# aquaskyline/SOAPdenovo-Trans

Hardware: AMD Instinct MI355X
Metric: pregraph k-mers hashed/sec (higher is better)
Workload: dtype u64

## Files before the change

soapdenovo-trans_amd/csrc/sdt_sk_scatter_seq.cuh:

```cuda
#pragma once
#include <hip/hip_runtime.h>
#include "sdt_kmer.cuh"
#include "sdt_table.cuh"
#include "sdt_superkmer.cuh"

using namespace sdt;

constexpr uint32_t SK_BLK = 128;
#ifndef SDT_SK_BLK2
#define SDT_SK_BLK2 1024
#endif
constexpr uint32_t SK_BLK2 = SDT_SK_BLK2;
constexpr uint32_t SK_DEAD = 0xFFFFFFFFu;

#ifdef SDT_SK_L2_LOG
extern __device__ unsigned long long *g_l2_log;
extern __device__ unsigned long long g_l2_log_cap;
__device__ inline void sk_log_alloc(uint32_t path, uint32_t end, uint32_t id)
{
	if (g_l2_log) {
		const unsigned long long at = atomicAdd(g_l2_log, 1ULL);
		if (at + 1 < g_l2_log_cap)
			g_l2_log[1 + at] = (1ULL << 63) | ((unsigned long long)path << 61) | ((unsigned long long)(threadIdx.x & 0x1FFF) << 48) |
			                   ((unsigned long long)(end & 0xFFFFFFu) << 24) | (unsigned long long)(id & 0xFFFFFFu);
	}
}
__device__ inline void sk_log_cursor(uint32_t kind, uint32_t lb, uint32_t chunk, uint32_t pos)
{
	if (g_l2_log) {
		const unsigned long long at = atomicAdd(g_l2_log, 1ULL);
		if (at + 1 < g_l2_log_cap)
			g_l2_log[1 + at] = (1ULL << 63) | (3ULL << 61) | ((unsigned long long)kind << 59) | ((unsigned long long)(blockIdx.x & 15u) << 55) |
			                   ((unsigned long long)(threadIdx.x & 1023u) << 45) | ((unsigned long long)(lb & 1023u) << 35) |
			                   ((unsigned long long)(pos > 31u ? 31u : pos) << 30) | (unsigned long long)(chunk & 0x3FFFFFFFu);
	}
}
#else
__device__ inline void sk_log_alloc(uint32_t, uint32_t, uint32_t) {}
__device__ inline void sk_log_cursor(uint32_t, uint32_t, uint32_t, uint32_t) {}
#endif

__device__ inline uint32_t sk_alloc_chunk(unsigned long long *s_blk, const SkPool &pool, uint32_t blk = SK_BLK)
{
	uint32_t got = 0;
	bool done = false;
	while (!done) {
		{
			const unsigned long long w = __hip_atomic_load(s_blk, __ATOMIC_RELAXED, __HIP_MEMORY_SCOPE_WORKGROUP);
			if ((uint32_t)w > (uint32_t)(w >> 32)) {
				__builtin_amdgcn_s_sleep(1);
				continue;
			}
		}
		const unsigned long long v = atomicAdd(s_blk, 1ULL);
		const uint32_t id = (uint32_t)v, end = (uint32_t)(v >> 32);
		if (id < end) {
			got = id;
			done = true;
			sk_log_alloc(0, end, id);
		} else if (id == end) {
			const uint32_t base = atomicAdd(pool.next, blk);
			atomicExch(s_blk, ((unsigned long long)(base + blk) << 32) | (unsigned long long)(base + 1u));
			got = base;
			done = true;
			sk_log_alloc(1, end, base);
		}
	}
	return got;
}

__device__ inline uint32_t sk_alloc_chunks(unsigned long long *s_blk, const SkPool &pool, uint32_t n, uint32_t blk)
{
	uint32_t got = SK_NOCHUNK;
	bool done = false;
	while (!done) {
		{
			const unsigned long long w = __hip_atomic_load(s_blk, __ATOMIC_RELAXED, __HIP_MEMORY_SCOPE_WORKGROUP);
			if ((uint32_t)w > (uint32_t)(w >> 32)) {
				__builtin_amdgcn_s_sleep(1);
				continue;
			}
		}
		const unsigned long long v = atomicAdd(s_blk, (unsigned long long)n);
		const uint32_t id = (uint32_t)v, end = (uint32_t)(v >> 32);
		if (id <= end && id + n <= end) {
			got = id;
			done = true;
		} else if (id <= end) {
			for (uint32_t x = id; x < end && x < pool.chunks; x++)
				pool.meta[x] = SK_DEAD;
			const uint32_t base = atomicAdd(pool.next, n + blk);
			atomicExch(s_blk, ((unsigned long long)(base + n + blk) << 32) | (unsigned long long)(base + n));
			got = base;
			done = true;
		}
	}
	return got;
}

__device__ inline void sk_retire_block(unsigned long long blk, const SkPool &pool)
{
	const uint32_t next = (uint32_t)blk, end = (uint32_t)(blk >> 32);
	for (uint32_t id = next; id < end && id < pool.chunks; id++)
		pool.meta[id] = SK_DEAD;
}

__device__ inline bool sk_reserve(unsigned long long *s_cur, unsigned long long *s_blk, uint32_t lb, uint32_t meta_bucket,
                                  uint32_t cap, const SkPool &pool, uint32_t *s_cnt, uint32_t &chunk, uint32_t &pos)
{
	bool done = false, ok = false;
	while (!done) {
		if ((uint32_t)__hip_atomic_load(&s_cur[lb], __ATOMIC_RELAXED, __HIP_MEMORY_SCOPE_WORKGROUP) > cap) {
			__builtin_amdgcn_s_sleep(1);
			continue;
		}
		const unsigned long long cur = atomicAdd(&s_cur[lb], 1ULL);
		pos = (uint32_t)cur;
		chunk = (uint32_t)(cur >> 32);
		if (pos < cap) {
			ok = chunk != SK_NOCHUNK;
			done = true;
			sk_log_cursor(0, lb, chunk, pos);
		} else if (pos == cap) {
			sk_log_cursor(1, lb, chunk, pos);
			uint32_t id = sk_alloc_chunk(s_blk, pool);
			if (id >= pool.chunks) {
				id = SK_NOCHUNK;
			} else {
				pool.meta[id] = meta_bucket | (cap << 24);
				atomicAdd(&s_cnt[lb], 1u);
			}
			atomicExch(&s_cur[lb], ((unsigned long long)id << 32) | 1ULL);
			chunk = id;
			pos = 0;
			ok = id != SK_NOCHUNK;
			done = true;
			sk_log_cursor(3, lb, id, 1);
		} else {
#if SDT_SK_L2_LOG >= 2
			sk_log_cursor(2, lb, chunk, pos);
#endif
		}
	}
	return ok;
}

template <int RW> __device__ inline void sk_store_record(uint64_t *dst, const uint64_t (&rec)[RW])
{
#pragma unroll
	for (int i = 0; i < RW; i++)
		dst[i] = rec[i];
}
template <int NW> __device__ inline void sk_store_record2(uint64_t *dst, const uint64_t (&rec)[SkFmt<NW>::REC_WORDS])
{
	if constexpr (SkFmt<NW>::REC2_STRIDE == 4 && SkFmt<NW>::REC_WORDS == 3) {
		ulonglong2 *d = reinterpret_cast<ulonglong2 *>(dst);
		d[0] = make_ulonglong2(rec[0], rec[1]);
		d[1] = make_ulonglong2(rec[2], 0ULL);
	} else {
		sk_store_record<SkFmt<NW>::REC_WORDS>(dst, rec);
	}
}
template <int RW> __device__ inline void sk_load_record(const uint64_t *src, uint64_t (&rec)[RW])
{
#pragma unroll
	for (int i = 0; i < RW; i++)
		rec[i] = src[i];
}


constexpr int SK_SEQ_TILE = 256;
constexpr int SK_SEQ_RUNCAP = 24;
constexpr int SK_SEQ_MAX_KMERS = 256;


template <int NW>
__device__ inline void sk_emit_run(const uint32_t *words, int rb_r, int len_r, int nk_r, int K, uint64_t read_ord, int j0, int n,
                                   uint32_t fb, unsigned long long *s_cur, unsigned long long *s_blk, const SkPool &pool,
                                   uint32_t *s_cnt, const Table<NW> &tbl, uint32_t &claimed, uint32_t &failed, uint32_t &done,
                                   uint32_t &emitted)
{
	constexpr int BW = SkFmt<NW>::BW, RW = SkFmt<NW>::REC_WORDS;
	const int hp = j0 > 0, hn = j0 + n < nk_r;
	const uint32_t l1 = fb >> SK_L2BITS, l2 = fb & (SK_NB2 - 1);
	uint32_t chunk, pos;
	if (sk_reserve(s_cur, s_blk, l1, l1, SK_CAP1, pool, s_cnt, chunk, pos)) {
		const int len = hp + n + K - 1 + hn, ps = rb_r + j0 - hp;
		uint64_t rec[RW];
		rec[0] = sk_header(read_ord, (uint32_t)j0, l2, n, hp, hn);
#pragma unroll
		for (int k = 0; k < BW; k++) {
			uint64_t wv = 0;
			if (32 * k < len) {
				wv = sk_stream_word(words, ps + 32 * k);
				const int keep = len - 32 * k;
				if (keep < 32)
					wv &= ~0ULL << (64 - 2 * keep);
			}
			rec[1 + k] = wv;
		}
		sk_store_record<RW>(pool.recs + ((size_t)chunk * SK_CAP1 + pos) * RW, rec);
		emitted += (uint32_t)n;
	} else if (!tbl.ent) {
		failed += (uint32_t)n;
	} else {
		for (int jj = j0; jj < j0 + n; jj++) {
			uint32_t prev, next;
			const Key<NW> key = chop_record<NW>(words, rb_r, len_r, jj, K, prev, next);
			const uint64_t ord = tbl.first ? (read_ord << 16) | (uint64_t)jj : ORD_NONE;
			if (!table_put<NW>(tbl, key, prev, next, claimed, ord))
				failed++;
			done++;
		}
	}
}

template <int NW, int W>
__global__ __launch_bounds__(SK_SEQ_TILE, NW == 1 ? 4 : 2) void k_sk_scatter_reads_seq(const uint32_t *__restrict__ packed, const uint64_t *__restrict__ offs,
                                                                      uint64_t nreads, int K, int m, int ncap, int max_tile_words, SkPool pool,
                                                                      unsigned long long *__restrict__ g_cursors, unsigned long long *__restrict__ g_blk,
                                                                      uint32_t *__restrict__ g_cnt, Table<NW> tbl, Stats *stats,
                                                                      uint64_t ord_base, uint64_t ord_stride)
{
	constexpr int TR = SK_SEQ_TILE;
	extern __shared__ uint32_t smem[];
	unsigned long long *s_cur = (unsigned long long *)smem;
	uint32_t *s_rb = (uint32_t *)(s_cur + SK_NB1);
	uint32_t *s_runs = s_rb + TR + 2;
	uint32_t *s_words = s_runs + TR * SK_SEQ_RUNCAP;
	__shared__ unsigned long long s_blk;
	__shared__ uint32_t s_cnt[SK_NB1];
	const int tid = threadIdx.x;
	for (int i = tid; i < SK_NB1; i += TR) {
		s_cur[i] = g_cursors[(size_t)blockIdx.x * SK_NB1 + i];
		s_cnt[i] = 0;
	}
	if (tid == 0)
		s_blk = g_blk[blockIdx.x];
	const uint64_t ntiles = (nreads + TR - 1) / TR;
	const uint32_t mmask = (1u << (2 * m)) - 1u;
	const int topsh = 2 * (m - 1);
	uint32_t claimed = 0, failed = 0, done = 0, emitted = 0;
#ifdef SDT_SK_TICKS
	unsigned long long cyc[4] = {0, 0, 0, 0}, t0 = wall_clock64(), t1;
#define SK_TICK(i) do { t1 = wall_clock64(); cyc[i] += t1 - t0; t0 = t1; } while (0)
#else
#define SK_TICK(i) do { } while (0)
#endif
	for (uint64_t tile = blockIdx.x; tile < ntiles; tile += gridDim.x) {
		const uint64_t r0 = tile * TR;
		const int nr = (int)((nreads - r0) < (uint64_t)TR ? (nreads - r0) : (uint64_t)TR);
		const uint64_t word0 = offs[r0] >> 4;
		int nwords = (int)(((offs[r0 + nr] + 15) >> 4) - word0) + TAIL_PAD;
		if (nwords > max_tile_words)
			nwords = max_tile_words;
		s_rb[tid] = (uint32_t)(offs[r0 + (tid < nr ? tid : nr)] - (word0 << 4));
		if (tid == 0)
			s_rb[TR] = (uint32_t)(offs[r0 + nr] - (word0 << 4));
		if (tid < LDS_LEAD)
			s_words[tid] = 0;
		for (int i = tid; i < nwords; i += TR)
			s_words[LDS_LEAD + i] = packed[word0 + i];
		__syncthreads();
		SK_TICK(0);
		const uint32_t *words = s_words + LDS_LEAD;
		const int rb_r = (int)s_rb[tid];
		const int len_r = tid < nr ? (int)s_rb[tid + 1] - rb_r : 0;
		const int nk_r = len_r >= K + 1 ? len_r - K + 1 : 0;
		const uint64_t read_ord = ord_base + (r0 + (uint64_t)tid) * ord_stride;
		uint32_t *runs = s_runs + tid * SK_SEQ_RUNCAP;
		int nrun = 0;
		if (nk_r > 0) {
			const int nhv = len_r - m + 1;
			uint32_t fw = sk_stream_mmer(words, rb_r, m) >> 2;
			uint32_t rc = (sk_rev2bit32(fw ^ 0xAAAAAAAAu) >> (32 - 2 * (m - 1))) << 2;
			int pb = rb_r + m - 1;
			auto next_hv = [&]() -> uint32_t {
				const uint32_t b = (words[pb >> 4] >> (30 - 2 * (pb & 15))) & 3u;
				pb++;
				fw = ((fw << 2) | b) & mmask;
				rc = (rc >> 2) | ((b ^ 2u) << topsh);
				return sk_mmer_hash(fw < rc ? fw : rc);
			};
			int j0 = 0;
			uint32_t fb0 = 0, pfb = 0;
			auto window = [&](int j, uint32_t mn) {
				const uint32_t fb = sk_final_bucket(sk_bucket_hash(mn));
				if (j == 0) {
					fb0 = fb;
				} else if (j - j0 >= ncap || fb != pfb) {
					if (nrun < SK_SEQ_RUNCAP)
						runs[nrun] = (fb0 << 6) | (uint32_t)(j - j0 - 1);
					else
						sk_emit_run<NW>(words, rb_r, len_r, nk_r, K, read_ord, j0, j - j0, fb0, s_cur, &s_blk, pool, s_cnt, tbl, claimed, failed, done, emitted);
					nrun++;
					j0 = j;
					fb0 = fb;
				}
				pfb = fb;
			};
			uint32_t h[W], nh[W];
#pragma clang loop unroll(full)
			for (int i = 0; i < W; i++)
				h[i] = next_hv();
#pragma clang loop unroll(full)
			for (int i = W - 2; i >= 0; i--)
				h[i] = h[i] < h[i + 1] ? h[i] : h[i + 1];
			int p = W;
			for (int jb = 0; jb < nk_r; jb += W) {
				window(jb, h[0]);
				uint32_t pre = 0xFFFFFFFFu;
#pragma clang loop unroll(full)
				for (int i = 1; i < W; i++) {
					const uint32_t x = p < nhv ? next_hv() : 0xFFFFFFFFu;
					p++;
					nh[i - 1] = x;
					pre = x < pre ? x : pre;
					if (jb + i < nk_r)
						window(jb + i, h[i] < pre ? h[i] : pre);
				}
				nh[W - 1] = p < nhv ? next_hv() : 0xFFFFFFFFu;
				p++;
				h[W - 1] = nh[W - 1];
#pragma clang loop unroll(full)
				for (int i = W - 2; i >= 0; i--)
					h[i] = nh[i] < h[i + 1] ? nh[i] : h[i + 1];
			}
			if (nrun < SK_SEQ_RUNCAP)
				runs[nrun] = (fb0 << 6) | (uint32_t)(nk_r - j0 - 1);
			else
				sk_emit_run<NW>(words, rb_r, len_r, nk_r, K, read_ord, j0, nk_r - j0, fb0, s_cur, &s_blk, pool, s_cnt, tbl, claimed, failed, done, emitted);
			nrun++;
		}
		SK_TICK(1);
		const int nlist = nrun < SK_SEQ_RUNCAP ? nrun : SK_SEQ_RUNCAP;
		for (int k = 0, jr = 0; k < nlist; k++) {
			const uint32_t e = runs[k];
			const int nr = (int)(e & 63u) + 1;
			sk_emit_run<NW>(words, rb_r, len_r, nk_r, K, read_ord, jr, nr, e >> 6, s_cur, &s_blk, pool, s_cnt, tbl, claimed, failed, done, emitted);
			jr += nr;
		}
		__syncthreads();
		SK_TICK(3);
	}
#undef SK_TICK
	for (int i = tid; i < SK_NB1; i += TR) {
		g_cursors[(size_t)blockIdx.x * SK_NB1 + i] = s_cur[i];
		if (s_cnt[i])
			atomicAdd(&g_cnt[i], s_cnt[i]);
	}
	if (tid == 0) {
		g_blk[blockIdx.x] = s_blk;
#ifdef SDT_SK_TICKS
		for (int i = 0; i < 4; i++)
			atomicAdd(&stats->sk_cyc1[i], cyc[i]);
#endif
	}
	if (done) {
		atomicAdd(&stats->kmers, (unsigned long long)done);
		atomicAdd(&stats->sk_direct, (unsigned long long)done);
	}
	if (claimed) atomicAdd(&stats->distinct, (unsigned long long)claimed);
	if (failed) atomicAdd(&stats->probe_fail, (unsigned long long)failed);
#pragma unroll
	for (int d = 32; d > 0; d >>= 1)
		emitted += __shfl_down(emitted, d);
	if ((tid & 63) == 0 && emitted)
		atomicAdd(&stats->sk_emitted, (unsigned long long)emitted);
}


struct SkSeqLaunch {
	const uint32_t *words;
	const uint64_t *offs;
	uint64_t nreads;
	int K, m, ncap, mtw;
	SkPool pool;
	unsigned long long *cursors, *blk;
	uint32_t *cnt;
	Stats *stats;
	uint64_t ord_base, ord_stride;
	unsigned max_wgs;
	int cu_count;
	hipStream_t stream;
};

template <int NW, int W> inline hipError_t sk_seq_launch_one(const SkSeqLaunch &a, const Table<NW> &tbl)
{
	const size_t smem = (size_t)SK_NB1 * 8 + (size_t)(SK_SEQ_TILE + 2) * 4 + (size_t)SK_SEQ_TILE * SK_SEQ_RUNCAP * 4 + (size_t)(LDS_LEAD + a.mtw) * 4;
	hipError_t e = hipFuncSetAttribute((const void *)k_sk_scatter_reads_seq<NW, W>, hipFuncAttributeMaxDynamicSharedMemorySize, (int)smem);
	if (e != hipSuccess) return e;
	int per_cu = 0;
	e = hipOccupancyMaxActiveBlocksPerMultiprocessor(&per_cu, k_sk_scatter_reads_seq<NW, W>, SK_SEQ_TILE, smem);
	if (e != hipSuccess) return e;
	uint64_t res = (uint64_t)(per_cu > 0 ? per_cu : 1) * (uint64_t)a.cu_count;
	if (res > a.max_wgs) res = a.max_wgs;
	const uint64_t nt = (a.nreads + SK_SEQ_TILE - 1) / SK_SEQ_TILE;
	const unsigned grid = (unsigned)(nt < res ? nt : res);
	hipLaunchKernelGGL((k_sk_scatter_reads_seq<NW, W>), dim3(grid), dim3(SK_SEQ_TILE), smem, a.stream, a.words, a.offs, a.nreads, a.K, a.m, a.ncap,
	                   a.mtw, a.pool, a.cursors, a.blk, a.cnt, tbl, a.stats, a.ord_base, a.ord_stride);
	return hipGetLastError();
}

hipError_t sk_seq_launch_nw1(int w, const SkSeqLaunch &a, const Table<1> &tbl);
hipError_t sk_seq_launch_nw2_lo(int w, const SkSeqLaunch &a, const Table<2> &tbl);
hipError_t sk_seq_launch_nw2_mid(int w, const SkSeqLaunch &a, const Table<2> &tbl);
hipError_t sk_seq_launch_nw2_hi(int w, const SkSeqLaunch &a, const Table<2> &tbl);
```

Measured before the change: 94.44 billion.

## Restructure super-k-mer walk with block base loads, 24-bit hash and warp-uniform windows

Reworks the per-read minimizer walk. Each block of W bases is now fetched with a few word loads and funnel shifts instead of one shared-memory load per base, and the m-mer hash is computed with 24-bit multiply-add instructions in inline assembly. The window loop uses a branch-free 'cut' scheme, with a full-block specialisation chosen when the whole warp agrees. Run-list overflow is handled by pausing the walk to flush the runs and then resuming, instead of emitting inline from inside the loop. The NW=2 launch bound is raised to 3 blocks per CU and the LDS tile is padded for over-reads, which may increase register pressure and changes the hash function's values.

```diff
diff --git a/soapdenovo-trans_amd/csrc/sdt_sk_scatter_seq.cuh b/soapdenovo-trans_amd/csrc/sdt_sk_scatter_seq.cuh
--- a/soapdenovo-trans_amd/csrc/sdt_sk_scatter_seq.cuh
+++ b/soapdenovo-trans_amd/csrc/sdt_sk_scatter_seq.cuh
@@ -1,5 +1,6 @@
 #pragma once
 #include <hip/hip_runtime.h>
+#include <type_traits>
 #include "sdt_kmer.cuh"
 #include "sdt_table.cuh"
 #include "sdt_superkmer.cuh"
@@ -172,6 +173,30 @@
 constexpr int SK_SEQ_TILE = 256;
 constexpr int SK_SEQ_RUNCAP = 24;
 constexpr int SK_SEQ_MAX_KMERS = 256;
+constexpr int SK_SEQ_OVERREAD = 4;
+
+template <int W> __device__ inline void sk_seq_block_bases(const uint32_t *words, int pb, uint32_t (&d)[(W + 15) / 16])
+{
+	constexpr int NO = (W + 15) / 16;
+	const int wi = pb >> 4, sh = 2 * (pb & 15);
+	uint32_t w[NO + 1];
+#pragma unroll
+	for (int k = 0; k <= NO; k++)
+		w[k] = words[wi + k];
+#pragma unroll
+	for (int k = 0; k < NO; k++)
+		d[k] = (uint32_t)(((((uint64_t)w[k] << 32) | w[k + 1]) << sh) >> 32);
+}
+
+__device__ inline uint32_t sk_mmer_hash24(uint32_t canon)
+{
+	constexpr uint32_t A = 0x7F4A7C15u, B = 0x9E3779B1u;
+	uint32_t up, lo;
+	asm("v_mul_u32_u24 %0, %1, %2" : "=v"(up) : "v"(canon), "s"(B >> 24));
+	asm("v_mad_u32_u24 %0, %1, %2, %3" : "=v"(lo) : "v"(canon), "s"(B & 0xFFFFFFu), "v"(A * B));
+	const uint32_t h = (up << 24) + lo;
+	return h ^ (h >> 15);
+}
 
 
 template <int NW>
@@ -216,7 +241,7 @@
 }
 
 template <int NW, int W>
-__global__ __launch_bounds__(SK_SEQ_TILE, NW == 1 ? 4 : 2) void k_sk_scatter_reads_seq(const uint32_t *__restrict__ packed, const uint64_t *__restrict__ offs,
+__global__ __launch_bounds__(SK_SEQ_TILE, NW == 1 ? 4 : 3) void k_sk_scatter_reads_seq(const uint32_t *__restrict__ packed, const uint64_t *__restrict__ offs,
                                                                       uint64_t nreads, int K, int m, int ncap, int max_tile_words, SkPool pool,
                                                                       unsigned long long *__restrict__ g_cursors, unsigned long long *__restrict__ g_blk,
                                                                       uint32_t *__restrict__ g_cnt, Table<NW> tbl, Stats *stats,
@@ -269,77 +294,100 @@
 		const int nk_r = len_r >= K + 1 ? len_r - K + 1 : 0;
 		const uint64_t read_ord = ord_base + (r0 + (uint64_t)tid) * ord_stride;
 		uint32_t *runs = s_runs + tid * SK_SEQ_RUNCAP;
-		int nrun = 0;
-		if (nk_r > 0) {
-			const int nhv = len_r - m + 1;
-			uint32_t fw = sk_stream_mmer(words, rb_r, m) >> 2;
-			uint32_t rc = (sk_rev2bit32(fw ^ 0xAAAAAAAAu) >> (32 - 2 * (m - 1))) << 2;
-			int pb = rb_r + m - 1;
-			auto next_hv = [&]() -> uint32_t {
-				const uint32_t b = (words[pb >> 4] >> (30 - 2 * (pb & 15))) & 3u;
-				pb++;
+		int nrun = 0, jr = 0;
+		bool walking = nk_r > 0;
+		uint32_t fw = 0, rc = 0, h[W], nh[W];
+		int pb = 0, jb = 0;
+		uint32_t fb0 = 0, s_fb0 = 0;
+		int cut = 0, s_cut = 0, nb = 0;
+		auto hash_block = [&](uint32_t (&out)[W]) {
+			uint32_t d[(W + 15) / 16];
+			sk_seq_block_bases<W>(words, pb, d);
+			pb += W;
+#pragma clang loop unroll(full)
+			for (int i = 0; i < W; i++) {
+				const uint32_t b = (d[i >> 4] >> (30 - 2 * (i & 15))) & 3u;
 				fw = ((fw << 2) | b) & mmask;
 				rc = (rc >> 2) | ((b ^ 2u) << topsh);
-				return sk_mmer_hash(fw < rc ? fw : rc);
-			};
-			int j0 = 0;
-			uint32_t fb0 = 0, pfb = 0;
-			auto window = [&](int j, uint32_t mn) {
-				const uint32_t fb = sk_final_bucket(sk_bucket_hash(mn));
-				if (j == 0) {
-					fb0 = fb;
-				} else if (j - j0 >= ncap || fb != pfb) {
-					if (nrun < SK_SEQ_RUNCAP)
-						runs[nrun] = (fb0 << 6) | (uint32_t)(j - j0 - 1);
-					else
-						sk_emit_run<NW>(words, rb_r, len_r, nk_r, K, read_ord, j0, j - j0, fb0, s_cur, &s_blk, pool, s_cnt, tbl, claimed, failed, done, emitted);
-					nrun++;
-					j0 = j;
-					fb0 = fb;
+				out[i] = sk_mmer_hash24(fw < rc ? fw : rc);
+			}
+		};
+		auto note = [&](int n) {
+			if ((uint32_t)nrun < (uint32_t)SK_SEQ_RUNCAP)
+				runs[nrun] = (fb0 << 6) | (uint32_t)(n - 1);
+			nrun++;
+		};
+		auto windows = [&](auto full) {
+			uint32_t pre = 0xFFFFFFFFu;
+#pragma clang loop unroll(full)
+			for (int i = 0; i < W; i++) {
+				if (i > 0)
+					pre = nh[i - 1] < pre ? nh[i - 1] : pre;
+				const uint32_t mn = h[i] < pre ? h[i] : pre;
+				if (decltype(full)::value || jb + i < nk_r) {
+					const uint32_t fb = sk_final_bucket(sk_bucket_hash(mn));
+					if (i >= cut || fb != fb0) {
+						note(i + ncap - cut);
+						cut = i + ncap;
+						fb0 = fb;
+					}
 				}
-				pfb = fb;
-			};
-			uint32_t h[W], nh[W];
-#pragma clang loop unroll(full)
-			for (int i = 0; i < W; i++)
-				h[i] = next_hv();
+			}
+		};
+		if (walking) {
+			fw = sk_stream_mmer(words, rb_r, m) >> 2;
+			rc = (sk_rev2bit32(fw ^ 0xAAAAAAAAu) >> (32 - 2 * (m - 1))) << 2;
+			pb = rb_r + m - 1;
+			hash_block(h);
 #pragma clang loop unroll(full)
 			for (int i = W - 2; i >= 0; i--)
 				h[i] = h[i] < h[i + 1] ? h[i] : h[i + 1];
-			int p = W;
-			for (int jb = 0; jb < nk_r; jb += W) {
-				window(jb, h[0]);
-				uint32_t pre = 0xFFFFFFFFu;
-#pragma clang loop unroll(full)
-				for (int i = 1; i < W; i++) {
-					const uint32_t x = p < nhv ? next_hv() : 0xFFFFFFFFu;
-					p++;
-					nh[i - 1] = x;
-					pre = x < pre ? x : pre;
-					if (jb + i < nk_r)
-						window(jb + i, h[i] < pre ? h[i] : pre);
+			hash_block(nh);
+			s_fb0 = sk_final_bucket(sk_bucket_hash(h[0]));
+			s_cut = ncap;
+		}
+		do {
+			int nemit = 0;
+			while (walking) {
+				cut = s_cut;
+				fb0 = s_fb0;
+				nrun = nb;
+				if (__all(jb + W <= nk_r))
+					windows(std::true_type());
+				else
+					windows(std::false_type());
+				const bool last = jb + W >= nk_r;
+				if (last)
+					note(nk_r - jb + ncap - cut);
+				if (nrun > SK_SEQ_RUNCAP) {
+					nemit = SK_SEQ_RUNCAP;
+					nb -= SK_SEQ_RUNCAP;
+					break;
 				}
-				nh[W - 1] = p < nhv ? next_hv() : 0xFFFFFFFFu;
-				p++;
+				if (last) {
+					nemit = nrun;
+					walking = false;
+					break;
+				}
+				s_cut = cut - W;
+				s_fb0 = fb0;
+				nb = nrun;
 				h[W - 1] = nh[W - 1];
 #pragma clang loop unroll(full)
 				for (int i = W - 2; i >= 0; i--)
 					h[i] = nh[i] < h[i + 1] ? nh[i] : h[i + 1];
-			}
-			if (nrun < SK_SEQ_RUNCAP)
-				runs[nrun] = (fb0 << 6) | (uint32_t)(nk_r - j0 - 1);
-			else
-				sk_emit_run<NW>(words, rb_r, len_r, nk_r, K, read_ord, j0, nk_r - j0, fb0, s_cur, &s_blk, pool, s_cnt, tbl, claimed, failed, done, emitted);
-			nrun++;
-		}
-		SK_TICK(1);
-		const int nlist = nrun < SK_SEQ_RUNCAP ? nrun : SK_SEQ_RUNCAP;
-		for (int k = 0, jr = 0; k < nlist; k++) {
-			const uint32_t e = runs[k];
-			const int nr = (int)(e & 63u) + 1;
-			sk_emit_run<NW>(words, rb_r, len_r, nk_r, K, read_ord, jr, nr, e >> 6, s_cur, &s_blk, pool, s_cnt, tbl, claimed, failed, done, emitted);
-			jr += nr;
-		}
+				jb += W;
+				hash_block(nh);
+			}
+			SK_TICK(1);
+			for (int k = 0; k < nemit; k++) {
+				const uint32_t e = runs[k];
+				const int nr = (int)(e & 63u) + 1;
+				sk_emit_run<NW>(words, rb_r, len_r, nk_r, K, read_ord, jr, nr, e >> 6, s_cur, &s_blk, pool, s_cnt, tbl, claimed, failed, done, emitted);
+				jr += nr;
+			}
+			SK_TICK(3);
+		} while (walking);
 		__syncthreads();
 		SK_TICK(3);
 	}
@@ -387,7 +435,8 @@
 
 template <int NW, int W> inline hipError_t sk_seq_launch_one(const SkSeqLaunch &a, const Table<NW> &tbl)
 {
-	const size_t smem = (size_t)SK_NB1 * 8 + (size_t)(SK_SEQ_TILE + 2) * 4 + (size_t)SK_SEQ_TILE * SK_SEQ_RUNCAP * 4 + (size_t)(LDS_LEAD + a.mtw) * 4;
+	const size_t smem = (size_t)SK_NB1 * 8 + (size_t)(SK_SEQ_TILE + 2) * 4 + (size_t)SK_SEQ_TILE * SK_SEQ_RUNCAP * 4 +
+	                    (size_t)(LDS_LEAD + a.mtw + SK_SEQ_OVERREAD) * 4;
 	hipError_t e = hipFuncSetAttribute((const void *)k_sk_scatter_reads_seq<NW, W>, hipFuncAttributeMaxDynamicSharedMemorySize, (int)smem);
 	if (e != hipSuccess) return e;
 	int per_cu = 0;
```

Result: faster. 96.80 billion (median of 6 runs) (+2.5%).
